# panuelosj/polystokes

Hardware: NVIDIA B200
Metric: stokes_steps_per_sec_256cubed (higher is better)
Workload: dtype f64

## Files before the change

### polystokes_b200/csrc/ps_api.cu

```cuda
#include "ps_solver.hpp"
#include <map>
#include <array>
#include <fstream>
#include <limits>
#include <thread>
#include <mutex>
#include <condition_variable>
#include <functional>
#include <memory>
#include <chrono>

using namespace ps;

struct MultiGroup;
struct ps_solver { Solver* S; void* tm[2] = {nullptr, nullptr}; Scratch scratch; MultiGroup* multi = nullptr; };

struct MultiGroup {
    struct Worker {
        std::thread th; std::mutex m; std::condition_variable cv;
        std::function<int()> task; bool has = false, quit = false, done = true; int rc = 0; std::string err;
        std::vector<void*> graveyard;
        const char* volatile where = "idle";
    };
    std::vector<ps_solver*> kids;
// ... 109 lines not shown
};
template <class Fn>
int guarded(ps_solver* h, Fn&& fn) {
    try { Enter e(h); return fn(); }
    catch (const std::exception& e) { g_lastError = e.what(); return PS_FAILED; }
    catch (...) { g_lastError = "unknown error"; return PS_FAILED; }
}

struct HostCsr { int64_t rows = 0, cols = 0; std::vector<int64_t> ptr; std::vector<int32_t> idx; std::vector<double> val; };

HostCsr diag_csr(const std::vector<double>& d) {
    HostCsr m; m.rows = m.cols = (int64_t)d.size(); m.ptr.resize(d.size() + 1); m.idx.resize(d.size()); m.val = d;
    for (size_t i = 0; i < d.size(); ++i) { m.ptr[i] = (int64_t)i; m.idx[i] = (int32_t)i; }
    m.ptr[d.size()] = (int64_t)d.size();
    return m;
}
HostCsr blockdiag_csr(const std::vector<double>& blocks, int R) {
    HostCsr m; m.rows = m.cols = (int64_t)R * RDOF;
    m.ptr.resize(m.rows + 1); m.idx.resize((size_t)R * RDOF * RDOF); m.val = blocks;
    for (int64_t r = 0; r <= m.rows; ++r) m.ptr[r] = r * RDOF;
    for (int b = 0; b < R; ++b) for (int i = 0; i < RDOF; ++i) for (int j = 0; j < RDOF; ++j) m.idx[((size_t)b * RDOF + i) * RDOF + j] = b * RDOF + j;
    return m;
}

HostCsr k_block(Solver& S, const std::string& name) {
    const Counts& C = S.C;
    const int64_t nRows = C.nRowsExt, nP = C.nPressures, nT = C.nStresses;
    std::vector<double> kv((size_t)8 * nRows); std::vector<int32_t> kc((size_t)8 * nRows);
    {
        std::vector<uint64_t> code = S.Op.kcode.to_host(S.st, (size_t)nRows);
        std::vector<int32_t> col = S.Op.kcol.to_host(S.st, (size_t)6 * nRows);
        const double sc = S.g.invDx / 64.;
        for (int64_t r = 0; r < nRows; ++r) {
            const int32_t c0w = col[r];
            const int64_t cOff = nP + (int64_t)((uint32_t)c0w >> 30) * C.nCenter;
            const int64_t c0 = c0w & OP_COL_MASK, c1 = col[(size_t)nRows + r];
            const int64_t cc[8] = {c0, c1, cOff + c0, cOff + c1, col[(size_t)2 * nRows + r], col[(size_t)3 * nRows + r], col[(size_t)4 * nRows + r], col[(size_t)5 * nRows + r]};
            for (int k = 0; k < 8; ++k) { kv[(size_t)k * nRows + r] = (double)op_code(code[r], k) * sc; kc[(size_t)k * nRows + r] = (int32_t)cc[k]; }
        }
    }
    const bool pressure = (name == "G" || name == "JG");
    const int64_t colLo = pressure ? 0 : nP, colHi = pressure ? nP : nP + nT;
    HostCsr m; m.cols = colHi - colLo;
    if (name == "G" || name == "Dt") {
        m.rows = C.nActiveVs; m.ptr.assign(m.rows + 1, 0);
        for (int64_t r = 0; r < m.rows; ++r) {
            std::vector<std::pair<int32_t, double>> e;
            for (int k = 0; k < 8; ++k) { const double v = kv[(size_t)k * nRows + r]; const int32_t c = kc[(size_t)k * nRows + r]; if (v != 0. && c >= colLo && c < colHi) e.push_back({(int32_t)(c - colLo), v}); }
            std::sort(e.begin(), e.end(), [](auto& a, auto& b) { return a.first < b.first; });
            for (auto& x : e) { m.idx.push_back(x.first); m.val.push_back(x.second); }
            m.ptr[r + 1] = (int64_t)m.idx.size();
        }
        return m;
    }
    const int R = S.RG.count;
    m.rows = (int64_t)R * RDOF; m.ptr.assign(m.rows + 1, 0);
    if (R == 0) return m;
    std::vector<int32_t> rowFace = S.RG.rowFace.to_host(S.st, (size_t)S.RG.nRows);
    std::vector<int32_t> rowStart = S.RG.rowStart.to_host(S.st, (size_t)R + 1);
    std::vector<double> com = S.RG.com.to_host(S.st, (size_t)3 * R);
    for (int r = 0; r < R; ++r) {
        std::map<int32_t, std::array<double, RDOF>> cols;
        for (int32_t row = rowStart[r]; row < rowStart[r + 1]; ++row) {
            const int32_t packed = rowFace[row];
            const int axis = (packed >> 29) & 3;
            const I3 f = delin(S.g, SL_FACE + axis, (int64_t)(packed & 0x1fffffff));
            double p[3] = {(double)f.x, (double)f.y, (double)f.z};
            p[axis] -= 0.5;
            double c[RDOF];
            conversion_coefficients(p[0] * S.g.dx - com[3 * r], p[1] * S.g.dx - com[3 * r + 1], p[2] * S.g.dx - com[3 * r + 2], axis, c);
// ... 499 lines not shown
```

### polystokes_b200/csrc/ps_assemble.cu

```cuda
#include "ps_solver.hpp"

namespace ps {

PS_D float local_viscosity_a(const Geom& g, const float* visc, int slot, const I3& idx) {
    int o[3] = {1, 1, 1};
    if (slot >= SL_FACE && slot < SL_EDGE) o[slot - SL_FACE] = 0;
    else if (slot >= SL_EDGE) { for (int a = 0; a < 3; ++a) if (a != slot - SL_EDGE) o[a] = 0; }
    const int b0 = o[0] ? idx.x : idx.x - 1, b1 = o[1] ? idx.y : idx.y - 1, b2 = o[2] ? idx.z : idx.z - 1;
    const float t0 = o[0] ? 0.f : 0.5f, t1 = o[1] ? 0.f : 0.5f, t2 = o[2] ? 0.f : 0.5f;
    float cz[2];
    for (int dz = 0; dz < 2; ++dz) {
        float cy[2];
        for (int dy = 0; dy < 2; ++dy) {
            const float a = float_at(g, visc, SL_CENTER, I3{b0, b1 + dy, b2 + dz});
            const float b = float_at(g, visc, SL_CENTER, I3{b0 + 1, b1 + dy, b2 + dz});
            cy[dy] = fadd_rn(a, fmul_rn(t0, fsub_rn(b, a)));
        }
        cz[dz] = fadd_rn(cy[0], fmul_rn(t1, fsub_rn(cy[1], cy[0])));
    }
    return fadd_rn(cz[0], fmul_rn(t2, fsub_rn(cz[1], cz[0])));
}

PS_D double clampd(double v, double lo, double hi) { return fmin(fmax(v, lo), hi); }

// ... 24 lines not shown
        ps_for_range(st, lo, hi, PS_LAMBDA(int64_t q) {
            const int64_t row = krow[q];
            if (row < 0 || !own.has(row)) return;
            const I3 f = delin(g, SL_FACE + axis, q);
            const int fw = ffw[q];
            uint64_t word = 0; int32_t c[6] = {0, 0, 0, 0, 0, 0};
            for (int dir = 0; dir < 2; ++dir) {
                const I3 cell = dir ? f : shifted(f, axis, -1);
                if (!in_bounds(g, SL_CENTER, cell)) continue;
                const int64_t qc = lin(g, SL_CENTER, cell);
                const int ci = CA[qc];
                if (ci < 0) continue;
                const int prod = fw * (int)clw[qc];
                if (prod <= 0) continue;
                word = pack_code(word, dir, dir ? prod : -prod);
                word = pack_code(word, 2 + dir, dir ? -prod : prod);
                c[dir] = ci;
            }
            for (int dir = 0; dir < 2; ++dir) {
                const I3 ed1 = dir ? shifted(f, 3 - axis - e1, 1) : f;
                const int64_t q1 = lin(g, SL_EDGE + e1, ed1);
                if (is_active(EL1[q1])) {
                    const int prod = fw * (int)ew1[q1];
                    if (prod > 0) { word = pack_code(word, 4 + dir, dir ? -prod : prod); c[2 + dir] = (int32_t)(eOff1 + EA1[q1]); }
                }
                const I3 ed2 = dir ? shifted(f, 3 - axis - e2, 1) : f;
                const int64_t q2 = lin(g, SL_EDGE + e2, ed2);
                if (is_active(EL2[q2])) {
                    const int prod = fw * (int)ew2[q2];
                    if (prod > 0) { word = pack_code(word, 6 + dir, dir ? -prod : prod); c[4 + dir] = (int32_t)(eOff2 + EA2[q2]); }
                }
            }
            kcode[row] = word;
            kcol[row] = c[0] | (int32_t)((uint32_t)axis << 30);
            for (int s = 1; s < 6; ++s) kcol[(int64_t)s * nRows + row] = c[s];
            if (row < nAct) {
                const double MINWEIGHT = 0.1;
                double volume = (double)fw * 0.125 * ((double)flw[q] * 0.125);
                volume = clampd(volume, MINWEIGHT * MINWEIGHT, 1.0);
                const double m = mul_rn(volume, density);
                const double lv = (double)vel[q];
                mc[row] = m; mcInv[row] = 1. / m;
                kmc[row] = (uint8_t)(fw * (int)flw[q]);
                rhsU[row] = mul_rn(mul_rn(lv, volume), density);
                oldVs[row] = lv;
            }
        });
    }
}

void k_assemble_Kt(cudaStream_t st, const Geom& g, const Fields& F, const Counts& C, CompactOp& Op, double* uInv, double* uDiag, double* rhsPT, bool ownOnly) {
    const int zA = ownOnly ? g.zLo : 0, zB = ownOnly ? g.zHi : g.nz;
    const int64_t nP = C.nPressures, nC = C.nCenter;
    const double invDx = g.invDx;
    const double MINWEIGHT = 0.1;
    {
        uint64_t* ccode = Op.ccode.p; int32_t* ccol = Op.ccol.p;
        const int32_t* CA = F.aidx[SL_CENTER];
        const uint8_t* clw = F.liqW[SL_CENTER]; const uint8_t* cfw = F.fluW[SL_CENTER];
        const int32_t* kr0 = F.krow[0]; const int32_t* kr1 = F.krow[1]; const int32_t* kr2 = F.krow[2];
        const uint8_t* fw0 = F.fluW[SL_FACE + 0]; const uint8_t* fw1 = F.fluW[SL_FACE + 1]; const uint8_t* fw2 = F.fluW[SL_FACE + 2];
        const float* cv0 = F.colvel[0]; const float* cv1 = F.colvel[1]; const float* cv2 = F.colvel[2];
        const float* visc = F.viscosity;
        const int64_t nAct = C.nActiveVs;
        int64_t lo, hi;
        z_range(g, SL_CENTER, zA, zB, lo, hi);
        ps_for_range(st, lo, hi, PS_LAMBDA(int64_t q) {
            const int ci = CA[q];
// ... 1 lines not shown
            const I3 c = delin(g, SL_CENTER, q);
            const int lw = clw[q], fwc = cfw[q];
            double rhsP = 0.;
            uint64_t word = 0; int32_t pcols[6];
            for (int axis = 0; axis < 3; ++axis) {
                const int32_t* kr = axis == 0 ? kr0 : axis == 1 ? kr1 : kr2;
                const uint8_t* fwA = axis == 0 ? fw0 : axis == 1 ? fw1 : fw2;
                const float* cvel = axis == 0 ? cv0 : axis == 1 ? cv1 : cv2;
                double rhsT = 0.;
                for (int side = 0; side < 2; ++side) {
                    const I3 f = side ? shifted(c, axis, 1) : c;
                    const int64_t qf = lin(g, SL_FACE + axis, f);
                    const int slot = axis * 2 + side;
                    pcols[slot] = 0;
                    const int64_t row = kr[qf];
                    if (row < 0) continue;
                    const int prod = (int)fwA[qf] * lw;
                    if (prod <= 0) continue;
                    const double coeff = pair_coeff(fwA[qf], lw, invDx);
                    const double sign = side ? -1. : 1.;
                    word = pack_code(word, slot, side ? -prod : prod);
                    pcols[slot] = (int32_t)row;
                    if (row < nAct) {
                        const double svel = (double)cvel[qf];
                        const double sc = sign * coeff;
                        if (fwc < 8) { rhsP += -1. * sc * svel; rhsT += -1. * sc * svel; }
                        if (fwA[qf] < 8) { rhsP += sc * svel; rhsT += sc * svel; }
                    }
                }
                const int64_t trow = (int64_t)axis * nC + ci;
                rhsPT[nP + trow] = rhsT;
            }
            ccode[ci] = word;
            for (int s = 0; s < 6; ++s) ccol[(int64_t)s * nC + ci] = pcols[s];
            rhsPT[ci] = rhsP;
            const double volumeWeight = clampd((double)fwc * 0.125, MINWEIGHT, 1.0) * ((double)lw * 0.125);
            const double localViscosity = (double)visc[q];
            const double invLocalViscosity = clampd(1. / localViscosity, 0., 1.e10);
            const double ui = mul_rn(invLocalViscosity, clampd(volumeWeight, 1.e-2, 1.));
            const double ud = mul_rn(localViscosity, clampd(1. / volumeWeight, 0., 1.e2));
            for (int axis = 0; axis < 3; ++axis) { uInv[(int64_t)axis * nC + ci] = ui; uDiag[(int64_t)axis * nC + ci] = ud; }
        });
    }
    const int64_t nERows = C.nEdge[0] + C.nEdge[1] + C.nEdge[2];
    for (int e = 0; e < 3; ++e) {
        uint32_t* ecode = Op.ecode.p; int32_t* ecol = Op.ecol.p;
        const int8_t* EL = F.label[SL_EDGE + e]; const int32_t* EA = F.aidx[SL_EDGE + e];
        const uint8_t* elw = F.liqW[SL_EDGE + e]; const uint8_t* efw = F.fluW[SL_EDGE + e];
        const int fa0 = (e == 0) ? 1 : 0, fa1 = (e == 2) ? 1 : 2;
        const int32_t* krA = F.krow[fa0]; const int32_t* krB = F.krow[fa1];
        const uint8_t* fwA = F.fluW[SL_FACE + fa0]; const uint8_t* fwB = F.fluW[SL_FACE + fa1];
        const float* cvA = F.colvel[fa0]; const float* cvB = F.colvel[fa1];
        const float* visc = F.viscosity;
        const int64_t eRowOff = C.stressOff[3 + e] - 3 * nC;
        const int64_t tOff = C.stressOff[3 + e];
        const int64_t nAct = C.nActiveVs;
        int64_t lo, hi;
        z_range(g, SL_EDGE + e, zA, zB, lo, hi);
        ps_for_range(st, lo, hi, PS_LAMBDA(int64_t q) {
            if (!is_active(EL[q])) return;
            const int ei = EA[q];
            const I3 ed = delin(g, SL_EDGE + e, q);
            const int lw = elw[q], fwe = efw[q];
            uint64_t word = 0; int32_t cidx[4] = {0, 0, 0, 0};
            double rhs = 0.;
            for (int k = 0; k < 4; ++k) {
                const int fa = k < 2 ? fa0 : fa1;
                const bool back = (k & 1) == 0;
                const I3 f = back ? shifted(ed, 3 - fa - e, -1) : ed;
                if (!in_bounds(g, SL_FACE + fa, f)) continue;
                const int64_t qf = lin(g, SL_FACE + fa, f);
                const int64_t row = (k < 2 ? krA : krB)[qf];
                if (row < 0) continue;
                const int ffw8 = (k < 2 ? fwA : fwB)[qf];
                const int prod = ffw8 * lw;
                if (prod <= 0) continue;
                const double coeff = pair_coeff(ffw8, lw, invDx);
                const double divSign = back ? 1. : -1.;
                word = pack_code(word, k, back ? -prod : prod);
                cidx[k] = (int32_t)row;
                if (row < nAct) {
                    const double svel = (double)(k < 2 ? cvA : cvB)[qf];
                    const double sc = divSign * coeff;
                    if (fwe < 8) rhs += -1. * sc * svel;
                    if (ffw8 < 8) rhs += sc * svel;
                }
            }
            const int64_t erow = eRowOff + ei;
            ecode[erow] = (uint32_t)word;
            for (int k = 0; k < 4; ++k) ecol[(int64_t)k * nERows + erow] = cidx[k];
            rhsPT[nP + tOff + ei] = rhs;
            const double volumeWeight = clampd((double)fwe * 0.125, MINWEIGHT, 1.0) * ((double)lw * 0.125);
            const double localViscosity = (double)local_viscosity_a(g, visc, SL_EDGE + e, ed);
            const double invLocalViscosity = clampd(1. / localViscosity, 0., 1e10);
            uInv[tOff + ei] = mul_rn(mul_rn(2., invLocalViscosity), volumeWeight);
            uDiag[tOff + ei] = mul_rn(mul_rn(0.5, localViscosity), clampd(1. / volumeWeight, 0., 1.e2));
        });
    }
}

}
```

### polystokes_b200/csrc/ps_explicit.cu

```cuda
#include "ps_solver.hpp"

namespace ps {

struct ExplCtx {
    OpArgs A;
    const int32_t* rowRegion; const uint32_t* rowXYZ; const double* com; const double* Binv;
    double dx, dt;
    const int32_t* regionOfCol;
    const int32_t* regStart;
    const int32_t* listCol;
    const int32_t* posOfCol;
    const double* VW;
};

PS_D int row_faces(const OpArgs& A, int64_t i, int64_t* f, double* val) {
    if (i < A.nP) {
        const uint64_t word = A.ccode[i];
        for (int k = 0; k < 6; ++k) { const int code = op_code(word, k); val[k] = (double)code * A.valScale; f[k] = code ? A.ccol[(int64_t)k * A.nC + i] : -1; }
        return 6;
    }
    const int64_t j = i - A.nP;
    if (j < 3 * A.nC) {
        const int a = (int)(j / A.nC); const int64_t ci = j - (int64_t)a * A.nC;
        const uint64_t word = A.ccode[ci];
        for (int k = 0; k < 2; ++k) { const int code = op_code(word, 2 * a + k); val[k] = -((double)code * A.valScale); f[k] = code ? A.ccol[(int64_t)(2 * a + k) * A.nC + ci] : -1; }
        return 2;
    }
    const int64_t e = j - 3 * A.nC;
    const uint32_t word = A.ecode[e];
    for (int k = 0; k < 4; ++k) { const int code = op_code(word, k); val[k] = (double)code * A.valScale; f[k] = code ? A.ecol[(int64_t)k * A.nE + e] : -1; }
    return 4;
}
PS_D void face_row_entries(const OpArgs& A, int64_t r, int64_t* col, double* val) {
    const uint64_t word = A.kcode[r];
    const int32_t c0w = A.kcol[r];
    const int64_t cOff = A.nP + (int64_t)((uint32_t)c0w >> 30) * A.nC;
    col[0] = c0w & OP_COL_MASK; col[1] = A.kcol[A.nRowsExt + r]; col[2] = cOff + col[0]; col[3] = cOff + col[1];
    for (int k = 0; k < 4; ++k) col[4 + k] = A.kcol[(int64_t)(2 + k) * A.nRowsExt + r];
    for (int k = 0; k < 8; ++k) val[k] = (double)op_code(word, k) * A.valScale;
}

constexpr int U_MAX = 49;
PS_D int build_u_list(const OpArgs& A, int64_t i, const int64_t* f, const double* kv, int ns, int32_t* ucol, double* uval) {
    int n = 0;
    auto insert = [&](int32_t c, double v) {
        int lo = 0;
        while (lo < n && ucol[lo] < c) ++lo;
        if (lo < n && ucol[lo] == c) { uval[lo] += v; return; }
        for (int q = n; q > lo; --q) { ucol[q] = ucol[q - 1]; uval[q] = uval[q - 1]; }
        ucol[lo] = c; uval[lo] = v; ++n;
    };
    for (int k = 0; k < ns; ++k) {
        if (kv[k] == 0. || f[k] >= A.nActiveVs) continue;
        int64_t col[8]; double val[8];
        face_row_entries(A, f[k], col, val);
        const double mcInv = A.mcInvLut[A.kmc[f[k]]];
        for (int s = 0; s < 8; ++s) if (val[s] != 0.) insert((int32_t)col[s], kv[k] * (mcInv * val[s]));
    }
    if (i >= A.nP) insert((int32_t)i, 0.);
    return n;
}

static void k_mark_region_columns(cudaStream_t st, const OpArgs& A, const int32_t* rowRegion, int32_t* regMax, int32_t* regMin) {
    ps_for(st, A.nRowsExt - A.nActiveVs, PS_LAMBDA(int64_t row) {
        int64_t col[8]; double val[8];
        face_row_entries(A, A.nActiveVs + row, col, val);
        const int r = rowRegion[row];
        for (int s = 0; s < 8; ++s) if (val[s] != 0.) { atomic_max(&regMax[col[s]], r); atomic_min(&regMin[col[s]], r); }
    });
}
static void k_region_column_flags(cudaStream_t st, int64_t n, const int32_t* regMax, int32_t* regMin, uint8_t* flag, int* conflict) {
// ... 123 lines not shown
```

### polystokes_b200/csrc/ps_pcg.cu

```cuda
#include "ps_solver.hpp"
#include "ps_peer.hpp"

namespace ps {

PS_D double k_row(const OpArgs& A, int64_t r, const double* __restrict__ x) {
    const uint64_t word = A.kcode[r];
    const int32_t c0w = A.kcol[r];
    const int64_t cOff = A.nP + (int64_t)((uint32_t)c0w >> 30) * A.nC;
    int64_t col[8];
    col[0] = c0w & OP_COL_MASK; col[1] = A.kcol[A.nRowsExt + r]; col[2] = cOff + col[0]; col[3] = cOff + col[1];
    for (int k = 0; k < 4; ++k) col[4 + k] = A.kcol[(int64_t)(2 + k) * A.nRowsExt + r];
    double s = 0.;
    for (int k = 0; k < 8; ++k) { const int code = op_code(word, k); if (code) s += ((double)code * A.valScale) * x[col[k]]; }
    return s;
}
PS_D void kt_cell_rows(const OpArgs& A, int64_t ci, const double* __restrict__ w, double* out) {
    const uint64_t word = A.ccode[ci];
    double v[6], wv[6];
    for (int k = 0; k < 6; ++k) { const int code = op_code(word, k); v[k] = (double)code * A.valScale; wv[k] = code ? w[A.ccol[(int64_t)k * A.nC + ci]] : 0.; }
    double s = 0.;
    for (int k = 0; k < 6; ++k) s += v[k] * wv[k];
    out[0] = s;
    for (int a = 0; a < 3; ++a) { double t = 0.; t += (-v[2 * a]) * wv[2 * a]; t += (-v[2 * a + 1]) * wv[2 * a + 1]; out[1 + a] = t; }
}
PS_D double kt_edge_row(const OpArgs& A, int64_t e, const double* __restrict__ w) {
    const uint64_t word = A.ecode[e];
    double s = 0.;
    for (int k = 0; k < 4; ++k) { const int code = op_code(word, k); if (code) s += ((double)code * A.valScale) * w[A.ecol[(int64_t)k * A.nE + e]]; }
    return s;
}

PS_D void moments_to_t(const double* M, double* t) {
    for (int n = 0; n < RDOF; ++n) t[n] = 0.;
    const double* A = M; const double* B = M + 10; const double* Cz = M + 20;
    t[0] = A[0]; t[3] = A[1]; t[4] = A[2]; t[5] = A[3]; for (int k = 0; k < 6; ++k) t[6 + k] = A[4 + k];
    t[1] = B[0]; t[12] = B[1]; t[13] = B[2]; t[14] = B[3]; for (int k = 0; k < 6; ++k) t[15 + k] = B[4 + k];
    t[2] += Cz[0]; t[3] += -Cz[3]; t[6] += -2. * Cz[6]; t[7] += -Cz[8]; t[8] += -0.5 * Cz[9];
    t[13] += -Cz[3]; t[16] += -Cz[6]; t[18] += -2. * Cz[8]; t[19] += -0.5 * Cz[9];
    t[21] += Cz[1]; t[22] += Cz[2]; t[23] += Cz[4]; t[24] += Cz[5]; t[25] += Cz[7];
}
PS_D void s_to_sigma(const double* s, double* sg) {
    sg[0] = s[0]; sg[1] = s[3]; sg[2] = s[4]; sg[3] = s[5]; for (int k = 0; k < 6; ++k) sg[4 + k] = s[6 + k];
    sg[10] = s[1]; sg[11] = s[12]; sg[12] = s[13]; sg[13] = s[14]; for (int k = 0; k < 6; ++k) sg[14 + k] = s[15 + k];
    double* z = sg + 20;
    z[0] = s[2]; z[1] = s[21]; z[2] = s[22]; z[3] = -s[3] - s[13]; z[4] = s[23]; z[5] = s[24];
    z[6] = -2. * s[6] - s[16]; z[7] = s[25]; z[8] = -s[7] - 2. * s[18]; z[9] = -0.5 * s[8] - 0.5 * s[19];
}

PS_D double sum_partials(const double* p, int n) { double s = 0.; for (int i = 0; i < n; ++i) s += p[i]; return s; }

PS_D double cg_rre2(double rr, double xx) { double rre = rr; if (rr / xx < rre) rre = rr / xx; return rre; }
PS_D double cg_next_xx(double xx, double alpha, double xp, double pp) { return xx + (2. * alpha) * xp + (alpha * alpha) * pp; }
PS_D double cg_next_rr(double rr, double alpha, double rAp, double ApAp) { return (rr - (2. * alpha) * rAp) + (alpha * alpha) * ApAp; }
PS_D double cg_r_new(double r, double alpha, double Ap) { return fma(-alpha, Ap, r); }
PS_D double cg_p_new(double rNew, double beta, double p) { return fma(beta, p, rNew); }
PS_D void cg_advance(PcgScalars* S, double rsold, double rr, double xx, double alpha, double pAp) {
    const double rre = cg_rre2(rr, xx);
    S->rsnew = rr; S->xmag = xx; S->xx = xx; S->rre = rre; S->pAp = pAp; S->alpha = alpha;
    if (rre < S->tol2) { S->done = 1; return; }
    S->beta = rr / rsold;
    S->rsold = rr;
// ... 29 lines not shown
    v = warp_sum(v);
    if ((threadIdx.x & 31) == 0) ws[threadIdx.x >> 5] = v;
    __syncthreads();
    double s = 0.;
    if (threadIdx.x < 32) { s = threadIdx.x < HOT_THREADS / 32 ? ws[threadIdx.x] : 0.; s = warp_sum(s); }
    __syncthreads();
    return s;
}
__device__ __forceinline__ double block_sum_partials(const double* p, int n) {
    double s = 0.;
    for (int i = threadIdx.x; i < n; i += HOT_THREADS) s += __ldcg(p + i);
    return block_sum(s);
}
__device__ __forceinline__ bool last_block(unsigned int* ticket) {
    __shared__ bool last;
    if (threadIdx.x == 0) {
        __threadfence();
        const unsigned t = atomicInc(ticket, gridDim.x - 1);
        last = (t == gridDim.x - 1);
        if (last) __threadfence();
    }
    __syncthreads();
    return last;
}

__device__ __forceinline__ void pass1_block(const OpArgs& A, const double* __restrict__ x, double* __restrict__ w, double activeScale, const double* lut, int32_t e) {
    const int k = (int)((uint32_t)e >> 28);
    const int64_t r = A.s1.lo[k] + (int64_t)(e & 0x0fffffff) * SCHED_BLOCK + threadIdx.x;
    if (r >= A.s1.hi[k]) return;
    const double sc = A.valScale;
    const uint64_t word = __ldcs(A.kcode + r);
    int32_t c[6];
#pragma unroll
    for (int k2 = 0; k2 < 6; ++k2) c[k2] = __ldcs(A.kcol + (int64_t)k2 * A.nRowsExt + r);
    const int64_t cOff = A.nP + (int64_t)((uint32_t)c[0] >> 30) * A.nC;
    const int64_t c0 = c[0] & OP_COL_MASK, c1 = c[1];
    const int64_t col[8] = {c0, c1, cOff + c0, cOff + c1, c[2], c[3], c[4], c[5]};
    double xv[8];
#pragma unroll
    for (int k2 = 0; k2 < 8; ++k2) xv[k2] = ((word >> (8 * k2)) & 0xffull) ? x[col[k2]] : 0.;
    double s = 0.;
#pragma unroll
    for (int k2 = 0; k2 < 8; ++k2) s += ((double)op_code(word, k2) * sc) * xv[k2];
    w[r] = r < A.nActiveVs ? activeScale * lut[__ldcs(A.kmc + r)] * s : s;
}
__global__ void __launch_bounds__(HOT_THREADS, 6) pass1_kernel(const __grid_constant__ OpArgs A, const double* __restrict__ x, double* __restrict__ w, double activeScale, const PcgScalars* S, int reverse,
                                                             const int32_t* __restrict__ sched, int nSched, const __grid_constant__ VecLink V) {    pdl_sync();

    __shared__ double lut[65];
    if (S && S->done) return;
    if (threadIdx.x < 65) lut[threadIdx.x] = A.mcInvLut[threadIdx.x];
    __syncthreads();
    if (!vec_wait(V)) { if (threadIdx.x == 0) const_cast<PcgScalars*>(S)->peerError = 1; return; }
#pragma unroll 2
    for (int g = blockIdx.x; g < nSched; g += gridDim.x) pass1_block(A, x, w, activeScale, lut, __ldg(sched + (reverse ? nSched - 1 - g : g)));
}
__device__ __forceinline__ void publish_partials(const PeerCtx& P, int slot, double v0, double v1, double v2) {
    __shared__ double pv[PEER_VALS];
    if (threadIdx.x == 0) { pv[0] = v0; pv[1] = v1; pv[2] = v2; }
    __syncthreads();
    const double vals[PEER_VALS] = {pv[0], pv[1], pv[2]};
    peer_reduce_push(P, slot, vals, PEER_VALS);
}
template <int OCC>
__global__ void __launch_bounds__(HOT_THREADS, OCC) pass2_kernel(const __grid_constant__ OpArgs A, const double* __restrict__ w, const double* __restrict__ x, double* __restrict__ y,
                                                              double muScale, const double* __restrict__ add, double* dotPartial, PcgScalars* S, int mode, const __grid_constant__ PeerCtx P,
                                                              const double* __restrict__ r2, int reverse, const __grid_constant__ VecLink V) {    pdl_sync();

    if (S && S->done) return;
    if (blockIdx.x == 0 && threadIdx.x == 0) vec_raise(V);
    if (!vec_wait(V)) { if (threadIdx.x == 0) S->peerError = 1; return; }
    const bool dot = mode & 1, dot3 = mode & 2;
    const double sc = A.valScale;
    const int64_t nC = A.nC, nP = A.nP, oE = A.nP + 3 * A.nC;
    double acc = 0., accR = 0., accY = 0.;
#pragma unroll 1
    for (int g = blockIdx.x; g < A.nSched2; g += gridDim.x) {
        const int32_t se = __ldg(A.sched2 + (reverse ? A.nSched2 - 1 - g : g));
        const int k = (int)((uint32_t)se >> 28);
        const int64_t row = A.s2.lo[k] + (int64_t)(se & 0x0fffffff) * SCHED_BLOCK + threadIdx.x;
        if (row >= A.s2.hi[k]) continue;
        if (k == 0) {
            const int64_t ci = row;
            const uint64_t word = __ldcs(A.ccode + ci);
            double v[6], wv[6];
#pragma unroll
            for (int q = 0; q < 6; ++q) {
                const int32_t c = __ldcs(A.ccol + (int64_t)q * nC + ci);
                v[q] = (double)op_code(word, q) * sc;
                wv[q] = ((word >> (8 * q)) & 0xffull) ? w[c] : 0.;
            }
            double s = 0.;
#pragma unroll
            for (int q = 0; q < 6; ++q) s += v[q] * wv[q];
            double yp = -s;
            if (add) yp += add[ci];
            y[ci] = yp;
            if (dot) acc += x[ci] * yp;
            if (dot3) { accR += r2[ci] * yp; accY += yp * yp; }
            const double ui = muScale != 0. ? muScale * A.uInv[ci] : 0.;
#pragma unroll
            for (int a = 0; a < 3; ++a) {
                double t = 0.;
                t += (-v[2 * a]) * wv[2 * a]; t += (-v[2 * a + 1]) * wv[2 * a + 1];
                const int64_t jj = nP + a * nC + ci;
                const double xj = x ? x[jj] : 0.;
                double yt = -t;
                if (muScale != 0.) yt -= ui * xj;
                if (add) yt += add[jj];
                y[jj] = yt;
                acc += xj * yt;
                if (dot3) { accR += r2[jj] * yt; accY += yt * yt; }
            }
        } else {
            const int64_t e = row;
            const uint32_t word = __ldcs(A.ecode + e);
            double s = 0.;
#pragma unroll
            for (int q = 0; q < 4; ++q) {
                const int32_t c = __ldcs(A.ecol + (int64_t)q * A.nE + e);
                const double wv = ((word >> (8 * q)) & 0xffu) ? w[c] : 0.;
                s += ((double)op_code(word, q) * sc) * wv;
            }
            const int64_t jj = oE + e;
            const double xj = x ? x[jj] : 0.;
            double yt = -s;
            if (muScale != 0.) yt -= muScale * A.uInv[3 * nC + e] * xj;
            if (add) yt += add[jj];
            y[jj] = yt;
            acc += xj * yt;
            if (dot3) { accR += r2[jj] * yt; accY += yt * yt; }
        }
    }
    if (dot) {
        const double bs = block_sum(acc);
        if (threadIdx.x == 0) dotPartial[blockIdx.x] = bs;
        if (dot3) {
            const double bR = block_sum(accR), bY = block_sum(accY);
            if (threadIdx.x == 0) { dotPartial[gridDim.x + blockIdx.x] = bR; dotPartial[2 * gridDim.x + blockIdx.x] = bY; }
        }
        if (last_block(&S->ticket[0])) {
            const double t = block_sum_partials(dotPartial, gridDim.x);
            double tR = 0., tY = 0.;
            if (dot3) { tR = block_sum_partials(dotPartial + gridDim.x, gridDim.x); tY = block_sum_partials(dotPartial + 2 * gridDim.x, gridDim.x); }
            if (threadIdx.x == 0) { S->red[0] = t; S->red[1] = tR; S->red[2] = tY; }
            if (P.nranks > 1) publish_partials(P, 0, t, tR, tY);
        }
    }
}
__global__ void __launch_bounds__(HOT_THREADS) cg_update_kernel(RangeSet own, double* __restrict__ x, double* __restrict__ r, double* __restrict__ p, const double* __restrict__ Ap,
                                                               double* dotPartial, PcgScalars* S, const __grid_constant__ PeerCtx P, int reverse, const __grid_constant__ VecLink V) {    pdl_sync();

    if (S->done) return;
    double a[3] = {S->red[0], S->red[1], S->red[2]}, b[3] = {S->red[3], S->red[4], S->red[5]};
// ... 414 lines not shown
    ps_for(st, 1, PS_LAMBDA(int64_t) {
        S->rhoCurr = 1.; S->rhoOld = 1.; S->alpha = 1.; S->beta = 0.; S->omega = 1.; S->xmag = 0.; S->rsnew = 0.; S->rre = 0.;
        S->bred[0] = 0.; S->bred[1] = 0.; S->tol = tol; S->tol2 = tol * tol; S->iter = 0; S->maxIter = maxIter; S->done = maxIter > 0 ? 0 : 2;
        S->ticket[6] = 0;
    });
}
void k_bicg_dot(cudaStream_t st, const RangeSet& own, const double* a0, const double* b0, const double* a1, const double* b1, double* dotPartial, PcgScalars* S) {
    if (a1) vec_sweep(st, own, dotPartial, S, 2, 0, true, PS_LAMBDA(int64_t i, double& a, double& b) { a += a0[i] * b0[i]; b += a1[i] * b1[i]; });
    else vec_sweep(st, own, dotPartial, S, 1, 0, true, PS_LAMBDA(int64_t i, double& a, double&) { a += a0[i] * b0[i]; });
}
void k_bicg_stage(cudaStream_t st, PcgScalars* S, int stage) { ps_for(st, 1, PS_LAMBDA(int64_t) { bicg_stage(S, stage); }); }
void k_bicg_update_p(cudaStream_t st, const RangeSet& own, double* p, const double* r, const double* v, const PcgScalars* S) {
    vec_sweep(st, own, nullptr, const_cast<PcgScalars*>(S), 0, 0, true, PS_LAMBDA(int64_t i, double&, double&) { p[i] = r[i] + S->beta * (p[i] - S->omega * v[i]); });
}
void k_bicg_update_hs(cudaStream_t st, const RangeSet& own, double* x, double* s, const double* r, const double* p, const double* v, const PcgScalars* S) {
    vec_sweep(st, own, nullptr, const_cast<PcgScalars*>(S), 0, 0, true, PS_LAMBDA(int64_t i, double&, double&) { const double al = S->alpha; x[i] = x[i] + al * p[i]; s[i] = r[i] - al * v[i]; });
}
void k_bicg_update_x(cudaStream_t st, const RangeSet& own, double* x, const double* s, double* dotPartial, PcgScalars* S) {
    vec_sweep(st, own, dotPartial, S, 1, 0, true, PS_LAMBDA(int64_t i, double& a, double&) { const double xi = x[i] + S->omega * s[i]; x[i] = xi; a += xi * xi; });
}
void k_bicg_err(cudaStream_t st, const RangeSet& own, const double* b, const double* Ax, double* dotPartial, PcgScalars* S) {
    vec_sweep(st, own, dotPartial, S, 1, 1, true, PS_LAMBDA(int64_t i, double& a, double&) { const double e = b[i] - Ax[i]; a += e * e; });
}
void k_bicg_update_r(cudaStream_t st, const RangeSet& own, double* r, const double* s, const double* t, const PcgScalars* S) {
    vec_sweep(st, own, nullptr, const_cast<PcgScalars*>(S), 0, 0, true, PS_LAMBDA(int64_t i, double&, double&) { r[i] = s[i] - S->omega * t[i]; });
}

void k_mark_K_columns(cudaStream_t st, const OpArgs& A, const RowSet& rows, const RangeSet& colsOwned, uint8_t* flag) {
    const RowSet R = rows; const RangeSet Cs = colsOwned;
    const uint64_t* kcode = A.kcode; const int32_t* kcol = A.kcol; const int64_t nRows = A.nRowsExt, nP = A.nP, nC = A.nC;
    ps_for(st, R.total(), PS_LAMBDA(int64_t l) {
        const int64_t r = R.at(l);
        const uint64_t word = kcode[r];
        const int32_t c0w = kcol[r];
        const int64_t cOff = nP + (int64_t)((uint32_t)c0w >> 30) * nC;
        int64_t col[8];
        col[0] = c0w & OP_COL_MASK; col[1] = kcol[nRows + r]; col[2] = cOff + col[0]; col[3] = cOff + col[1];
        for (int k = 0; k < 4; ++k) col[4 + k] = kcol[(int64_t)(2 + k) * nRows + r];
        for (int k = 0; k < 8; ++k) if (op_code(word, k) && Cs.has(col[k])) flag[col[k]] = 1;
    });
}
void k_mark_Kt_columns(cudaStream_t st, const OpArgs& A, const RowSet& cellRows, const RowSet& edgeRows, const RowSet& colsOwned, uint8_t* flag) {
    const RowSet Rc = cellRows, Re = edgeRows, Cs = colsOwned;
    const uint64_t* ccode = A.ccode; const int32_t* ccol = A.ccol; const uint32_t* ecode = A.ecode; const int32_t* ecol = A.ecol;
    const int64_t nC = A.nC, nE = A.nE;
    ps_for(st, Rc.total(), PS_LAMBDA(int64_t l) {
        const int64_t ci = Rc.at(l);
        const uint64_t word = ccode[ci];
        for (int k = 0; k < 6; ++k) { const int32_t c = ccol[(int64_t)k * nC + ci]; if (op_code(word, k) && Cs.has(c)) flag[c] = 1; }
    });
    ps_for(st, Re.total(), PS_LAMBDA(int64_t l) {
        const int64_t e = Re.at(l);
        const uint64_t word = ecode[e];
        for (int k = 0; k < 4; ++k) { const int32_t c = ecol[(int64_t)k * nE + e]; if (op_code(word, k) && Cs.has(c)) flag[c] = 1; }
    });
}

#ifndef PS_EMULATE
constexpr int RED_THREADS = 256;
constexpr int MOM_THREADS = 64;
__device__ __forceinline__ void region_solve(int r, int lane, const int32_t* __restrict__ chunkStart, const int32_t* __restrict__ chunk, const double* partial,
                                             const double* __restrict__ Binv, const double* __restrict__ extra, double extraScale, double tScale,
                                             double* tOut, double* sOut, double* __restrict__ sigma, double* M, double* t, double* sv) {
    if (lane < 30) {
        const int axis = lane / 10, k = lane % 10;
        double s = 0.;
        if (tScale != 0.)
            for (int ch = chunkStart[r]; ch < chunkStart[r + 1]; ++ch) if (chunk[4 * ch + 3] == axis) s += __ldcg(partial + (size_t)ch * 10 + k);
        M[lane] = s;
    }
    __syncthreads();
    if (lane == 0) moments_to_t(M, t);
    __syncthreads();
    if (lane < RDOF) {
        double v = tScale * t[lane];
        if (extra) v += extraScale * extra[(size_t)r * RDOF + lane];
        t[lane] = v; if (tOut) tOut[(size_t)r * RDOF + lane] = v;
    }
    __syncthreads();
    if (lane < RDOF) {
        const double* B = Binv + (size_t)r * RDOF * RDOF + lane * RDOF;
        double s = 0.;
#pragma unroll
        for (int j = 0; j < RDOF; ++j) s += B[j] * t[j];
        sv[lane] = s; if (sOut) sOut[(size_t)r * RDOF + lane] = s;
    }
    __syncthreads();
// ... 366 lines not shown

struct DiagCtx { const int32_t* rowRegion; const uint32_t* rowXYZ; const double* com; const double* Binv; double dx, dt; };
template <int NS>
PS_D double diag_row(const OpArgs& A, const DiagCtx& D, const int64_t* f, const double* val) {
    double uni = 0., red = 0.;
    bool used[NS];
    for (int k = 0; k < NS; ++k) {
        used[k] = (val[k] == 0.) || f[k] < A.nActiveVs;
        if (val[k] != 0. && f[k] < A.nActiveVs) uni += val[k] * val[k] * A.mcInvLut[A.kmc[f[k]]];
    }
    for (int k = 0; k < NS; ++k) {
        if (used[k]) continue;
        const int region = D.rowRegion[f[k] - A.nActiveVs];
        double V[RDOF], c[RDOF], m[10];
        for (int n = 0; n < RDOF; ++n) V[n] = 0.;
        for (int q = k; q < NS; ++q) {
            if (used[q] || D.rowRegion[f[q] - A.nActiveVs] != region) continue;
            used[q] = true;
            const uint32_t packed = D.rowXYZ[f[q] - A.nActiveVs];
            row_monomials(D.dx, packed, D.com + 3 * region, m);
            conversion_coefficients(m[1], m[2], m[3], (int)(packed >> 30), c);
            for (int n = 0; n < RDOF; ++n) V[n] += val[q] * c[n];
        }
        const double* B = D.Binv + (size_t)region * RDOF * RDOF;
        for (int i = 0; i < RDOF; ++i) { double t = 0.; for (int j = 0; j < RDOF; ++j) t += B[i * RDOF + j] * V[j]; red += V[i] * t; }
    }
    return -D.dt * uni - red;
}
void k_diag_A(cudaStream_t st, const Geom& g, const OpArgs& A, const RegionData& RG, double* diag) {
    const DiagCtx D = {RG.rowRegion.p, RG.rowXYZ.p, RG.com.p, RG.Binv.p, g.dx, g.dt};
    ps_for(st, A.nC, PS_LAMBDA(int64_t ci) {
        const uint64_t word = A.ccode[ci];
        int64_t f[6]; double v[6];
        for (int k = 0; k < 6; ++k) { const int code = op_code(word, k); v[k] = (double)code * A.valScale; f[k] = code ? A.ccol[(int64_t)k * A.nC + ci] : 0; }
        diag[ci] = diag_row<6>(A, D, f, v);
        for (int a = 0; a < 3; ++a) {
            const double va[2] = {-v[2 * a], -v[2 * a + 1]};
            const int64_t j = (int64_t)a * A.nC + ci;
            diag[A.nP + j] = diag_row<2>(A, D, f + 2 * a, va) - 0.5 * A.uInv[j];
        }
    });
    ps_for(st, A.nE, PS_LAMBDA(int64_t e) {
        const uint32_t word = A.ecode[e];
        int64_t f[4]; double v[4];
        for (int k = 0; k < 4; ++k) { const int code = op_code(word, k); v[k] = (double)code * A.valScale; f[k] = code ? A.ecol[(int64_t)k * A.nE + e] : 0; }
        const int64_t j = 3 * A.nC + e;
        diag[A.nP + j] = diag_row<4>(A, D, f, v) - 0.5 * A.uInv[j];
    });
}
void k_sigma_from_s(cudaStream_t st, int32_t R, const double* s, double* sigma) {
    ps_for(st, R, PS_LAMBDA(int64_t r) { double sg[30]; s_to_sigma(s + r * RDOF, sg); for (int k = 0; k < 30; ++k) sigma[r * 30 + k] = sg[k]; });
}
void k_guess_finish(cudaStream_t st, const OpArgs& A, double* guess) {
    ps_for(st, A.nT, PS_LAMBDA(int64_t i) { guess[A.nP + i] = (-2. * A.uInv[i]) * guess[A.nP + i]; });
}
PS_D double eig_invdiag(double d) { return d != 0. ? 1. / d : 1.; }
PS_D void eig_stage(PcgScalars* S, int stage) {
    if (S->done) return;
    if (stage == 0) {
        const double rhsNorm2 = S->bred[0], residualNorm2 = S->bred[1];
        S->eigRhsNorm2 = rhsNorm2;
        if (rhsNorm2 == 0.) { S->rre = 0.; S->done = 3; return; }
        const double t = S->tol * S->tol * rhsNorm2;
        S->eigThreshold = t > 2.2250738585072014e-308 ? t : 2.2250738585072014e-308;
        S->rre = sqrt(residualNorm2 / rhsNorm2);
        if (residualNorm2 < S->eigThreshold) S->done = 1;
        else if (S->maxIter <= 0) S->done = 2;
    } else if (stage == 1) {
        S->eigAbsNew = S->bred[0];
    } else {
        const double residualNorm2 = S->bred[0];
        S->rsnew = residualNorm2; S->rre = sqrt(residualNorm2 / S->eigRhsNorm2);
        if (residualNorm2 < S->eigThreshold) { S->done = 1; return; }
        const double absOld = S->eigAbsNew;
        S->eigAbsNew = S->bred[1];
        S->beta = S->eigAbsNew / absOld;
        S->iter += 1;
        if (S->iter >= S->maxIter) S->done = 2;
// ... 78 lines not shown
```

### polystokes_b200/csrc/ps_solver.hpp

```cpp
#pragma once
#include "ps_grid.hpp"
#include "ps_part.hpp"
#include "ps_comm.hpp"
#include "ps_peer.hpp"
#include "../../include/polystokes_b200.h"

namespace ps {

struct CompactOp {
    int64_t nRows = 0, nCells = 0, nEdges = 0;
    DBuf<uint64_t> kcode;
    DBuf<int32_t> kcol;
    DBuf<uint8_t> kmc;
    DBuf<double> mcInvLut;
    DBuf<uint64_t> ccode;
    DBuf<int32_t> ccol;
    DBuf<uint32_t> ecode;
    DBuf<int32_t> ecol;
    void alloc(int64_t rows, int64_t nAct, int64_t cells, int64_t edges) {
        nRows = rows; nCells = cells; nEdges = edges;
        kcode.alloc((size_t)rows + 1); kcol.alloc((size_t)6 * rows + 1); kmc.alloc((size_t)nAct + 1); mcInvLut.alloc(65);
        ccode.alloc((size_t)cells + 1); ccol.alloc((size_t)6 * cells + 1); ecode.alloc((size_t)edges + 1); ecol.alloc((size_t)4 * edges + 1);
    }
};
PS_HD int op_code(uint64_t word, int k) { return (int)(int8_t)(uint8_t)(word >> (8 * k)); }
constexpr int32_t OP_COL_MASK = 0x3fffffff;

constexpr int SCHED_BLOCK = 256;
struct SchedRanges {
    int n = 0;
    int64_t lo[4] = {0, 0, 0, 0}, hi[4] = {0, 0, 0, 0};
    int64_t items[4] = {-1, -1, -1, -1};
    void add(int64_t a, int64_t b) { lo[n] = a; hi[n] = b > a ? b : a; ++n; }
    void addItems(int64_t first, int64_t count) { lo[n] = first; hi[n] = first + (count > 0 ? count : 0); items[n] = count > 0 ? count : 0; ++n; }
    int64_t blocks(int k) const { return items[k] >= 0 ? items[k] : (hi[k] - lo[k] + SCHED_BLOCK - 1) / SCHED_BLOCK; }
};
std::vector<int32_t> merge_schedule(const SchedRanges& R);

struct RegionData {
    int32_t count = 0;
    DBuf<double> com;
    DBuf<double> Mr, Visc, N, Binv;
    DBuf<double> lsqRhs, bestFit, rhsR;
    DBuf<double> moments;
    DBuf<double> tables;
    DBuf<int32_t> cellList;
    DBuf<int32_t> cellStart;
    int64_t nRows = 0;
    DBuf<int32_t> rowFace;
    DBuf<uint32_t> rowXYZ;
    DBuf<double> sigma;
    DBuf<int32_t> rowRegion;
    DBuf<int32_t> rowStart;
    int32_t nCellChunks = 0, nRowChunks = 0;
    DBuf<int32_t> cellChunk;
    DBuf<int32_t> rowChunk;
    DBuf<int32_t> cellChunkStart, rowChunkStart;
    DBuf<int32_t> rowAxisStart;
    int32_t maxRegionRows = 0;
// ... 277 lines not shown
```

Measured before the change: 7.630.

## Interleave column index pairs so hot kernels load them as int2

```diff
diff --git a/polystokes_b200/csrc/ps_api.cu b/polystokes_b200/csrc/ps_api.cu
--- a/polystokes_b200/csrc/ps_api.cu
+++ b/polystokes_b200/csrc/ps_api.cu
@@ -165,10 +165,10 @@
         std::vector<int32_t> col = S.Op.kcol.to_host(S.st, (size_t)6 * nRows);
         const double sc = S.g.invDx / 64.;
         for (int64_t r = 0; r < nRows; ++r) {
-            const int32_t c0w = col[r];
+            const int32_t c0w = col[op_col_at(0, r, nRows)];
             const int64_t cOff = nP + (int64_t)((uint32_t)c0w >> 30) * C.nCenter;
-            const int64_t c0 = c0w & OP_COL_MASK, c1 = col[(size_t)nRows + r];
-            const int64_t cc[8] = {c0, c1, cOff + c0, cOff + c1, col[(size_t)2 * nRows + r], col[(size_t)3 * nRows + r], col[(size_t)4 * nRows + r], col[(size_t)5 * nRows + r]};
+            const int64_t c0 = c0w & OP_COL_MASK, c1 = col[op_col_at(1, r, nRows)];
+            const int64_t cc[8] = {c0, c1, cOff + c0, cOff + c1, col[op_col_at(2, r, nRows)], col[op_col_at(3, r, nRows)], col[op_col_at(4, r, nRows)], col[op_col_at(5, r, nRows)]};
             for (int k = 0; k < 8; ++k) { kv[(size_t)k * nRows + r] = (double)op_code(code[r], k) * sc; kc[(size_t)k * nRows + r] = (int32_t)cc[k]; }
         }
     }
diff --git a/polystokes_b200/csrc/ps_assemble.cu b/polystokes_b200/csrc/ps_assemble.cu
--- a/polystokes_b200/csrc/ps_assemble.cu
+++ b/polystokes_b200/csrc/ps_assemble.cu
@@ -80,8 +80,8 @@
                 }
             }
             kcode[row] = word;
-            kcol[row] = c[0] | (int32_t)((uint32_t)axis << 30);
-            for (int s = 1; s < 6; ++s) kcol[(int64_t)s * nRows + row] = c[s];
+            kcol[op_col_at(0, row, nRows)] = c[0] | (int32_t)((uint32_t)axis << 30);
+            for (int s = 1; s < 6; ++s) kcol[op_col_at(s, row, nRows)] = c[s];
             if (row < nAct) {
                 const double MINWEIGHT = 0.1;
                 double volume = (double)fw * 0.125 * ((double)flw[q] * 0.125);
@@ -149,7 +149,7 @@
                 rhsPT[nP + trow] = rhsT;
             }
             ccode[ci] = word;
-            for (int s = 0; s < 6; ++s) ccol[(int64_t)s * nC + ci] = pcols[s];
+            for (int s = 0; s < 6; ++s) ccol[op_col_at(s, ci, nC)] = pcols[s];
             rhsPT[ci] = rhsP;
             const double volumeWeight = clampd((double)fwc * 0.125, MINWEIGHT, 1.0) * ((double)lw * 0.125);
             const double localViscosity = (double)visc[q];
@@ -205,7 +205,7 @@
             }
             const int64_t erow = eRowOff + ei;
             ecode[erow] = (uint32_t)word;
-            for (int k = 0; k < 4; ++k) ecol[(int64_t)k * nERows + erow] = cidx[k];
+            for (int k = 0; k < 4; ++k) ecol[op_col_at(k, erow, nERows)] = cidx[k];
             rhsPT[nP + tOff + ei] = rhs;
             const double volumeWeight = clampd((double)fwe * 0.125, MINWEIGHT, 1.0) * ((double)lw * 0.125);
             const double localViscosity = (double)local_viscosity_a(g, visc, SL_EDGE + e, ed);
diff --git a/polystokes_b200/csrc/ps_explicit.cu b/polystokes_b200/csrc/ps_explicit.cu
--- a/polystokes_b200/csrc/ps_explicit.cu
+++ b/polystokes_b200/csrc/ps_explicit.cu
@@ -16,27 +16,27 @@
 PS_D int row_faces(const OpArgs& A, int64_t i, int64_t* f, double* val) {
     if (i < A.nP) {
         const uint64_t word = A.ccode[i];
-        for (int k = 0; k < 6; ++k) { const int code = op_code(word, k); val[k] = (double)code * A.valScale; f[k] = code ? A.ccol[(int64_t)k * A.nC + i] : -1; }
+        for (int k = 0; k < 6; ++k) { const int code = op_code(word, k); val[k] = (double)code * A.valScale; f[k] = code ? A.ccol[op_col_at(k, i, A.nC)] : -1; }
         return 6;
     }
     const int64_t j = i - A.nP;
     if (j < 3 * A.nC) {
         const int a = (int)(j / A.nC); const int64_t ci = j - (int64_t)a * A.nC;
         const uint64_t word = A.ccode[ci];
-        for (int k = 0; k < 2; ++k) { const int code = op_code(word, 2 * a + k); val[k] = -((double)code * A.valScale); f[k] = code ? A.ccol[(int64_t)(2 * a + k) * A.nC + ci] : -1; }
+        for (int k = 0; k < 2; ++k) { const int code = op_code(word, 2 * a + k); val[k] = -((double)code * A.valScale); f[k] = code ? A.ccol[op_col_at(2 * a + k, ci, A.nC)] : -1; }
         return 2;
     }
     const int64_t e = j - 3 * A.nC;
     const uint32_t word = A.ecode[e];
-    for (int k = 0; k < 4; ++k) { const int code = op_code(word, k); val[k] = (double)code * A.valScale; f[k] = code ? A.ecol[(int64_t)k * A.nE + e] : -1; }
+    for (int k = 0; k < 4; ++k) { const int code = op_code(word, k); val[k] = (double)code * A.valScale; f[k] = code ? A.ecol[op_col_at(k, e, A.nE)] : -1; }
     return 4;
 }
 PS_D void face_row_entries(const OpArgs& A, int64_t r, int64_t* col, double* val) {
     const uint64_t word = A.kcode[r];
-    const int32_t c0w = A.kcol[r];
+    const int32_t c0w = A.kcol[op_col_at(0, r, A.nRowsExt)];
     const int64_t cOff = A.nP + (int64_t)((uint32_t)c0w >> 30) * A.nC;
-    col[0] = c0w & OP_COL_MASK; col[1] = A.kcol[A.nRowsExt + r]; col[2] = cOff + col[0]; col[3] = cOff + col[1];
-    for (int k = 0; k < 4; ++k) col[4 + k] = A.kcol[(int64_t)(2 + k) * A.nRowsExt + r];
+    col[0] = c0w & OP_COL_MASK; col[1] = A.kcol[op_col_at(1, r, A.nRowsExt)]; col[2] = cOff + col[0]; col[3] = cOff + col[1];
+    for (int k = 0; k < 4; ++k) col[4 + k] = A.kcol[op_col_at(2 + k, r, A.nRowsExt)];
     for (int k = 0; k < 8; ++k) val[k] = (double)op_code(word, k) * A.valScale;
 }
 
diff --git a/polystokes_b200/csrc/ps_pcg.cu b/polystokes_b200/csrc/ps_pcg.cu
--- a/polystokes_b200/csrc/ps_pcg.cu
+++ b/polystokes_b200/csrc/ps_pcg.cu
@@ -5,11 +5,11 @@
 
 PS_D double k_row(const OpArgs& A, int64_t r, const double* __restrict__ x) {
     const uint64_t word = A.kcode[r];
-    const int32_t c0w = A.kcol[r];
+    const int32_t c0w = A.kcol[op_col_at(0, r, A.nRowsExt)];
     const int64_t cOff = A.nP + (int64_t)((uint32_t)c0w >> 30) * A.nC;
     int64_t col[8];
-    col[0] = c0w & OP_COL_MASK; col[1] = A.kcol[A.nRowsExt + r]; col[2] = cOff + col[0]; col[3] = cOff + col[1];
-    for (int k = 0; k < 4; ++k) col[4 + k] = A.kcol[(int64_t)(2 + k) * A.nRowsExt + r];
+    col[0] = c0w & OP_COL_MASK; col[1] = A.kcol[op_col_at(1, r, A.nRowsExt)]; col[2] = cOff + col[0]; col[3] = cOff + col[1];
+    for (int k = 0; k < 4; ++k) col[4 + k] = A.kcol[op_col_at(2 + k, r, A.nRowsExt)];
     double s = 0.;
     for (int k = 0; k < 8; ++k) { const int code = op_code(word, k); if (code) s += ((double)code * A.valScale) * x[col[k]]; }
     return s;
@@ -17,7 +17,7 @@
 PS_D void kt_cell_rows(const OpArgs& A, int64_t ci, const double* __restrict__ w, double* out) {
     const uint64_t word = A.ccode[ci];
     double v[6], wv[6];
-    for (int k = 0; k < 6; ++k) { const int code = op_code(word, k); v[k] = (double)code * A.valScale; wv[k] = code ? w[A.ccol[(int64_t)k * A.nC + ci]] : 0.; }
+    for (int k = 0; k < 6; ++k) { const int code = op_code(word, k); v[k] = (double)code * A.valScale; wv[k] = code ? w[A.ccol[op_col_at(k, ci, A.nC)]] : 0.; }
     double s = 0.;
     for (int k = 0; k < 6; ++k) s += v[k] * wv[k];
     out[0] = s;
@@ -26,7 +26,7 @@
 PS_D double kt_edge_row(const OpArgs& A, int64_t e, const double* __restrict__ w) {
     const uint64_t word = A.ecode[e];
     double s = 0.;
-    for (int k = 0; k < 4; ++k) { const int code = op_code(word, k); if (code) s += ((double)code * A.valScale) * w[A.ecol[(int64_t)k * A.nE + e]]; }
+    for (int k = 0; k < 4; ++k) { const int code = op_code(word, k); if (code) s += ((double)code * A.valScale) * w[A.ecol[op_col_at(k, e, A.nE)]]; }
     return s;
 }
 
@@ -122,7 +122,7 @@
     const uint64_t word = __ldcs(A.kcode + r);
     int32_t c[6];
 #pragma unroll
-    for (int k2 = 0; k2 < 6; ++k2) c[k2] = __ldcs(A.kcol + (int64_t)k2 * A.nRowsExt + r);
+    for (int k2 = 0; k2 < 3; ++k2) { const int2 cc = __ldcs(reinterpret_cast<const int2*>(A.kcol) + (int64_t)k2 * A.nRowsExt + r); c[2 * k2] = cc.x; c[2 * k2 + 1] = cc.y; }
     const int64_t cOff = A.nP + (int64_t)((uint32_t)c[0] >> 30) * A.nC;
     const int64_t c0 = c[0] & OP_COL_MASK, c1 = c[1];
     const int64_t col[8] = {c0, c1, cOff + c0, cOff + c1, c[2], c[3], c[4], c[5]};
@@ -174,11 +174,13 @@
             const int64_t ci = row;
             const uint64_t word = __ldcs(A.ccode + ci);
             double v[6], wv[6];
+            int32_t c[6];
+#pragma unroll
+            for (int q = 0; q < 3; ++q) { const int2 cc = __ldcs(reinterpret_cast<const int2*>(A.ccol) + (int64_t)q * nC + ci); c[2 * q] = cc.x; c[2 * q + 1] = cc.y; }
 #pragma unroll
             for (int q = 0; q < 6; ++q) {
-                const int32_t c = __ldcs(A.ccol + (int64_t)q * nC + ci);
                 v[q] = (double)op_code(word, q) * sc;
-                wv[q] = ((word >> (8 * q)) & 0xffull) ? w[c] : 0.;
+                wv[q] = ((word >> (8 * q)) & 0xffull) ? w[c[q]] : 0.;
             }
             double s = 0.;
 #pragma unroll
@@ -206,10 +208,12 @@
             const int64_t e = row;
             const uint32_t word = __ldcs(A.ecode + e);
             double s = 0.;
+            int32_t c[4];
+#pragma unroll
+            for (int q = 0; q < 2; ++q) { const int2 cc = __ldcs(reinterpret_cast<const int2*>(A.ecol) + (int64_t)q * A.nE + e); c[2 * q] = cc.x; c[2 * q + 1] = cc.y; }
 #pragma unroll
             for (int q = 0; q < 4; ++q) {
-                const int32_t c = __ldcs(A.ecol + (int64_t)q * A.nE + e);
-                const double wv = ((word >> (8 * q)) & 0xffu) ? w[c] : 0.;
+                const double wv = ((word >> (8 * q)) & 0xffu) ? w[c[q]] : 0.;
                 s += ((double)op_code(word, q) * sc) * wv;
             }
             const int64_t jj = oE + e;
@@ -690,11 +694,11 @@
     ps_for(st, R.total(), PS_LAMBDA(int64_t l) {
         const int64_t r = R.at(l);
         const uint64_t word = kcode[r];
-        const int32_t c0w = kcol[r];
+        const int32_t c0w = kcol[op_col_at(0, r, nRows)];
         const int64_t cOff = nP + (int64_t)((uint32_t)c0w >> 30) * nC;
         int64_t col[8];
-        col[0] = c0w & OP_COL_MASK; col[1] = kcol[nRows + r]; col[2] = cOff + col[0]; col[3] = cOff + col[1];
-        for (int k = 0; k < 4; ++k) col[4 + k] = kcol[(int64_t)(2 + k) * nRows + r];
+        col[0] = c0w & OP_COL_MASK; col[1] = kcol[op_col_at(1, r, nRows)]; col[2] = cOff + col[0]; col[3] = cOff + col[1];
+        for (int k = 0; k < 4; ++k) col[4 + k] = kcol[op_col_at(2 + k, r, nRows)];
         for (int k = 0; k < 8; ++k) if (op_code(word, k) && Cs.has(col[k])) flag[col[k]] = 1;
     });
 }
@@ -705,12 +709,12 @@
     ps_for(st, Rc.total(), PS_LAMBDA(int64_t l) {
         const int64_t ci = Rc.at(l);
         const uint64_t word = ccode[ci];
-        for (int k = 0; k < 6; ++k) { const int32_t c = ccol[(int64_t)k * nC + ci]; if (op_code(word, k) && Cs.has(c)) flag[c] = 1; }
+        for (int k = 0; k < 6; ++k) { const int32_t c = ccol[op_col_at(k, ci, nC)]; if (op_code(word, k) && Cs.has(c)) flag[c] = 1; }
     });
     ps_for(st, Re.total(), PS_LAMBDA(int64_t l) {
         const int64_t e = Re.at(l);
         const uint64_t word = ecode[e];
-        for (int k = 0; k < 4; ++k) { const int32_t c = ecol[(int64_t)k * nE + e]; if (op_code(word, k) && Cs.has(c)) flag[c] = 1; }
+        for (int k = 0; k < 4; ++k) { const int32_t c = ecol[op_col_at(k, e, nE)]; if (op_code(word, k) && Cs.has(c)) flag[c] = 1; }
     });
 }
 
@@ -1143,7 +1147,7 @@
     ps_for(st, A.nC, PS_LAMBDA(int64_t ci) {
         const uint64_t word = A.ccode[ci];
         int64_t f[6]; double v[6];
-        for (int k = 0; k < 6; ++k) { const int code = op_code(word, k); v[k] = (double)code * A.valScale; f[k] = code ? A.ccol[(int64_t)k * A.nC + ci] : 0; }
+        for (int k = 0; k < 6; ++k) { const int code = op_code(word, k); v[k] = (double)code * A.valScale; f[k] = code ? A.ccol[op_col_at(k, ci, A.nC)] : 0; }
         diag[ci] = diag_row<6>(A, D, f, v);
         for (int a = 0; a < 3; ++a) {
             const double va[2] = {-v[2 * a], -v[2 * a + 1]};
@@ -1154,7 +1158,7 @@
     ps_for(st, A.nE, PS_LAMBDA(int64_t e) {
         const uint32_t word = A.ecode[e];
         int64_t f[4]; double v[4];
-        for (int k = 0; k < 4; ++k) { const int code = op_code(word, k); v[k] = (double)code * A.valScale; f[k] = code ? A.ecol[(int64_t)k * A.nE + e] : 0; }
+        for (int k = 0; k < 4; ++k) { const int code = op_code(word, k); v[k] = (double)code * A.valScale; f[k] = code ? A.ecol[op_col_at(k, e, A.nE)] : 0; }
         const int64_t j = 3 * A.nC + e;
         diag[A.nP + j] = diag_row<4>(A, D, f, v) - 0.5 * A.uInv[j];
     });
diff --git a/polystokes_b200/csrc/ps_solver.hpp b/polystokes_b200/csrc/ps_solver.hpp
--- a/polystokes_b200/csrc/ps_solver.hpp
+++ b/polystokes_b200/csrc/ps_solver.hpp
@@ -25,6 +25,7 @@
 };
 PS_HD int op_code(uint64_t word, int k) { return (int)(int8_t)(uint8_t)(word >> (8 * k)); }
 constexpr int32_t OP_COL_MASK = 0x3fffffff;
+PS_HD int64_t op_col_at(int slot, int64_t row, int64_t n) { return (int64_t)(slot >> 1) * 2 * n + 2 * row + (slot & 1); }
 
 constexpr int SCHED_BLOCK = 256;
 struct SchedRanges {
```

New measurement: 7.713, median of 6. 1.01x the previous value.
